# ChristianFeldmann/libHM

Hardware: AMD Instinct MI355X
Metric: decoded Mpixels/s (luma), 2160p Main10 reconstruction + loop filters (higher is better)
Workload: dtype int16 samples / int32 accumulate; 1 GPU; 3840x2160 Main10 lowdelay_P pictures, pre-parsed CTU metadata: prep+MC+dequant/IT/recon+deblock+SAO, batch of 16 independent pictures per step, inputs resident in HBM; sub_benchmark=full, streams=2, parallelism=frame-parallel, 1 process per GPU, no data-path collective

## Files before the change

libhm_amd/csrc/itx_core.h:

```cpp
#pragma once
#include "hmgpu_dev.h"

namespace hmgpu {

__host__ __device__ constexpr int cos64(int a) {
  constexpr int t[33] = {64, 90, 90, 90, 89, 88, 87, 85, 83, 82, 80, 78, 75, 73, 70, 67, 64,
                         61, 57, 54, 50, 46, 43, 38, 36, 31, 25, 22, 18, 13, 9,  4,  0};
  return t[a];
}
__host__ __device__ constexpr int tmat(int n_size, int k, int n) {
  const int a = ((2 * n + 1) * k * (32 / n_size)) & 127;
  return a <= 32 ? cos64(a) : (a <= 64 ? -cos64(64 - a) : (a <= 96 ? -cos64(a - 64) : cos64(128 - a)));
}
__host__ __device__ constexpr int dst4(int m, int k) {
  constexpr int t[4][4] = {{29, 55, 74, 84}, {74, 74, 0, -74}, {84, -29, -74, 55}, {55, -84, 74, -29}};
  return t[m][k];
}

__device__ inline void wave_lds_sync() {
  __builtin_amdgcn_fence(__ATOMIC_RELEASE, "wavefront");
  __builtin_amdgcn_wave_barrier();
  __builtin_amdgcn_fence(__ATOMIC_ACQUIRE, "wavefront");
}

typedef short short2v __attribute__((ext_vector_type(2)));
__host__ __device__ constexpr uint32_t pkc(int lo, int hi) { return ((uint32_t)lo & 0xffffu) | ((uint32_t)hi << 16); }

__host__ __device__ constexpr int slot_k(int n_size, int s) {
  int size = n_size / 2, g = 1, base = 0;
  while (size >= 1) {
    if (s < base + size) return (2 * (s - base) + 1) << (g - 1);
    base += size; size /= 2; g++;
  }
  return 0;
}
__host__ __device__ constexpr int slot_of_c(int n_size, int k) {
  for (int s = 0; s < n_size; s++) if (slot_k(n_size, s) == k) return s;
  return -1;
}
__device__ inline int slot_of(int n_size, int k) {
  if (k == 0) return n_size - 1;
  const int g = __builtin_ctz(k) + 1;
  return n_size - (n_size >> (g - 1)) + (k >> g);
}

__device__ inline int dot2c(uint32_t pair, uint32_t taps, int acc) {
  return __builtin_amdgcn_sdot2(__builtin_bit_cast(short2v, pair), __builtin_bit_cast(short2v, taps), acc, false);
}
__device__ inline int dot2_z(uint32_t pair, uint32_t taps) {
  int d;
  asm("v_dot2_i32_i16 %0, %1, %2, 0" : "=v"(d) : "v"(pair), "s"(taps));
  return d;
}
__device__ inline int dot2_v(uint32_t pair, uint32_t taps, int seed) {
  int d;
  asm("v_dot2_i32_i16 %0, %1, %2, %3" : "=v"(d) : "v"(pair), "s"(taps), "v"(seed));
  return d;
}
__device__ inline uint32_t pk_mad_sat(uint32_t a, uint32_t b) {
  uint32_t d;
  asm("v_pk_mad_i16 %0, %1, %2, 0 clamp" : "=v"(d) : "v"(a), "v"(b));
  return d;
}
__device__ inline uint32_t pk_add_sat(uint32_t a, uint32_t b) {
  uint32_t d;
  asm("v_pk_add_i16 %0, %1, %2 clamp" : "=v"(d) : "v"(a), "v"(b));
  return d;
}
__device__ inline uint32_t cvt_pk_sat(int lo, int hi) {
  uint32_t d;
  asm("v_cvt_pk_i16_i32 %0, %1, %2" : "=v"(d) : "v"(lo), "v"(hi));
  return d;
}
__device__ inline uint32_t pk_clip_u(uint32_t v, uint32_t hi) {
  const short2v z = {0, 0};
  const short2v r = __builtin_elementwise_min(__builtin_elementwise_max(__builtin_bit_cast(short2v, v), z), __builtin_bit_cast(short2v, hi));
  return __builtin_bit_cast(uint32_t, r);
}

template <int N, int OFF, int NP>
__device__ inline void idct_pk(const uint32_t (&p)[NP], int seed, int (&out)[N]) {
  if constexpr (N == 2) {
    out[0] = dot2_v(p[OFF], pkc(64, 64), seed);
    out[1] = dot2_v(p[OFF], pkc(-64, 64), seed);
  } else {
    int e[N / 2];
    idct_pk<N / 2, OFF + N / 4, NP>(p, seed, e);
#pragma unroll
    for (int m = 0; m < N / 2; m++) {
      int o = dot2_z(p[OFF], pkc(tmat(N, 1, m), tmat(N, 3, m)));
#pragma unroll
      for (int i = 1; i < N / 4; i++) o = dot2c(p[OFF + i], pkc(tmat(N, 4 * i + 1, m), tmat(N, 4 * i + 3, m)), o);
      out[m] = e[m] + o;
      out[N - 1 - m] = e[m] - o;
    }
  }
}

template <int LOG2N> struct PkCfg {
  static constexpr int N = 1 << LOG2N;
  static constexpr int S = N == 4 ? 4 : (N == 8 ? 24 : N + 8);
  static constexpr int TU_ELEMS = N * S + (N >= 16 ? 8 : 0);
  static constexpr int TPB = 256 / N;
};

template <int N, int S>
__device__ inline void scatter_row(int16_t* __restrict__ buf, int sn, const uint32_t (&v)[N / 2]) {
#pragma unroll
  for (int i = 0; i < N / 2; i++) {
    buf[(2 * i) * S + sn] = (int16_t)(v[i] & 0xffffu);
    buf[(2 * i + 1) * S + sn] = (int16_t)(v[i] >> 16);
  }
}
template <int N, int S>
__device__ inline void gather_row(const int16_t* __restrict__ buf, int n, uint32_t (&v)[N / 2]) {
  if constexpr (N == 4) {
    const u32x2 a = *reinterpret_cast<const u32x2*>(buf + n * S);
    v[0] = a.x; v[1] = a.y;
  } else {
#pragma unroll
    for (int i = 0; i < N / 8; i++) {
      const u32x4 a = *reinterpret_cast<const u32x4*>(buf + n * S + 8 * i);
      v[4 * i] = a.x; v[4 * i + 1] = a.y; v[4 * i + 2] = a.z; v[4 * i + 3] = a.w;
    }
  }
}
__device__ inline int half_of(uint32_t w, int hi) { return hi ? ((int)w >> 16) : (int)(int16_t)(w & 0xffffu); }

template <int N>
__device__ inline void idst4_pk(const uint32_t (&p)[N / 2], int seed, int (&out)[N]) {
  if constexpr (N == 4) {
#pragma unroll
    for (int k = 0; k < 4; k++) out[k] = dot2c(p[1], pkc(dst4(2, k), dst4(0, k)), dot2_v(p[0], pkc(dst4(1, k), dst4(3, k)), seed));
  }
}
template <int LOG2N>
__device__ inline void itx_tu_pk(const uint32_t (&lv)[(1 << LOG2N) / 2], int n, int per, int rem, bool skip, int bd,
                                 int16_t* __restrict__ buf, uint32_t (&res)[(1 << LOG2N) / 2], bool dst = false,
                                 const uint8_t* __restrict__ mrow = nullptr, bool bypass = false) {
  constexpr int N = 1 << LOG2N, S = PkCfg<LOG2N>::S;
  if (bypass) {
#pragma unroll
    for (int i = 0; i < N / 2; i++) res[i] = lv[i];
    return;
  }
  const int tshift = 15 - bd - LOG2N;
  const int rshift = 6 - (tshift + per);
  const int scale = rem == 0 ? 40 : rem == 1 ? 45 : rem == 2 ? 51 : rem == 3 ? 57 : rem == 4 ? 64 : 72;
  uint32_t d[N / 2];
  if (mrow != nullptr) {
    const int rs = rshift + 4;
    const int tb = min(16, 17 + rs), in_max = (1 << (tb - 1)) - 1, in_min = -in_max - 1;
    uint32_t mw[N / 4];
    if constexpr (N == 4) mw[0] = ldg(reinterpret_cast<const uint32_t*>(mrow));
    else {
#pragma unroll
      for (int i = 0; i < N / 16; i++) { const u32x4 a = ldg4(mrow + 16 * i); mw[4 * i] = a.x; mw[4 * i + 1] = a.y; mw[4 * i + 2] = a.z; mw[4 * i + 3] = a.w; }
      if constexpr (N == 8) { const u32x2 a = ldg2(mrow); mw[0] = a.x; mw[1] = a.y; }
    }
#pragma unroll
    for (int i = 0; i < N / 2; i++) {
      const int m0 = (mw[i / 2] >> (16 * (i & 1))) & 0xff, m1 = (mw[i / 2] >> (16 * (i & 1) + 8)) & 0xff;
      const int q0 = clip3(in_min, in_max, half_of(lv[i], 0)), q1 = clip3(in_min, in_max, half_of(lv[i], 1));
      int c0 = __mul24(q0, scale * m0), c1 = __mul24(q1, scale * m1);
      if (rs > 0) { c0 = (c0 + (1 << (rs - 1))) >> rs; c1 = (c1 + (1 << (rs - 1))) >> rs; }
      else { c0 = (int)((unsigned)c0 << (-rs)); c1 = (int)((unsigned)c1 << (-rs)); }
      d[i] = cvt_pk_sat(c0, c1);
    }
  } else if (rshift <= 0) {
    const uint32_t sp = (uint32_t)(scale << (-rshift)) * 0x10001u;
#pragma unroll
    for (int i = 0; i < N / 2; i++) d[i] = pk_mad_sat(lv[i], sp);
  } else {
    const int add = 1 << (rshift - 1);
#pragma unroll
    for (int i = 0; i < N / 2; i++)
      d[i] = cvt_pk_sat((__mul24(half_of(lv[i], 0), scale) + add) >> rshift, (__mul24(half_of(lv[i], 1), scale) + add) >> rshift);
  }
  const int sn = slot_of(N, n);
  scatter_row<N, S>(buf, sn, d);
  wave_lds_sync();
  uint32_t p[N / 2];
  gather_row<N, S>(buf, n, p);
  wave_lds_sync();
  uint32_t t1[N / 2];
  if (skip) {
    int o[N];
#pragma unroll
    for (int sidx = 0; sidx < N; sidx++) {
      const int c = half_of(p[sidx / 2], sidx & 1);
      o[slot_k(N, sidx)] = tshift > 0 ? (c + (1 << (tshift - 1))) >> tshift : (tshift == 0 ? c : c << (-tshift));
    }
#pragma unroll
    for (int i = 0; i < N / 2; i++) t1[i] = cvt_pk_sat(o[2 * i], o[2 * i + 1]);
  } else {
    int o[N];
    if (LOG2N == 2 && dst) idst4_pk<N>(p, 64, o);
    else idct_pk<N, 0, N / 2>(p, 64, o);
#pragma unroll
    for (int i = 0; i < N / 2; i++) t1[i] = cvt_pk_sat(o[2 * i] >> 7, o[2 * i + 1] >> 7);
  }
  scatter_row<N, S>(buf, sn, t1);
  wave_lds_sync();
  uint32_t q[N / 2];
  gather_row<N, S>(buf, n, q);
  wave_lds_sync();
  if (skip) {
#pragma unroll
    for (int i = 0; i < N / 2; i++) {
      constexpr int dummy = 0; (void)dummy;
      const int s0 = slot_of_c(N, 2 * i), s1 = slot_of_c(N, 2 * i + 1);
      res[i] = __builtin_amdgcn_perm(q[s1 / 2], q[s0 / 2], ((s1 & 1) ? 0x07060000u : 0x05040000u) | ((s0 & 1) ? 0x0302u : 0x0100u));
    }
  } else {
    const int shift2 = 20 - bd;
    int r[N];
    if (LOG2N == 2 && dst) idst4_pk<N>(q, 1 << (shift2 - 1), r);
    else idct_pk<N, 0, N / 2>(q, 1 << (shift2 - 1), r);
#pragma unroll
    for (int i = 0; i < N / 2; i++) res[i] = cvt_pk_sat(r[2 * i] >> shift2, r[2 * i + 1] >> shift2);
  }
}

template <int LOG2N>
__device__ inline void resid_rotate_rdpcm(uint32_t (&res)[(1 << LOG2N) / 2], int n, bool rotate, int rdpcm) {
  constexpr int N = 1 << LOG2N;
  typedef unsigned short u16x2 __attribute__((ext_vector_type(2)));
  if constexpr (N == 4) {
    if (rotate) {
      const uint32_t a = (uint32_t)__shfl_xor((int)res[1], 3), b = (uint32_t)__shfl_xor((int)res[0], 3);
      res[0] = (a >> 16) | (a << 16); res[1] = (b >> 16) | (b << 16);
    }
  }
  if (rdpcm == 1) {
    uint32_t carry = 0;
#pragma unroll
    for (int i = 0; i < N / 2; i++) {
      const uint32_t lo = (res[i] + carry) & 0xffffu, hi = ((res[i] >> 16) + lo) & 0xffffu;
      res[i] = lo | (hi << 16); carry = hi;
    }
  } else if (rdpcm == 2) {
#pragma unroll
    for (int d = 1; d < N; d <<= 1) {
#pragma unroll
      for (int i = 0; i < N / 2; i++) {
        const uint32_t up = (uint32_t)__shfl_up((int)res[i], d, N);
        const u16x2 s = __builtin_bit_cast(u16x2, res[i]) + __builtin_bit_cast(u16x2, up);
        if (n >= d) res[i] = __builtin_bit_cast(uint32_t, s);
      }
    }
  }
}

}
```

libhm_amd/csrc/k_itx.hip:

```cpp
#include "hmgpu_dev.h"
#include "itx_core.h"
#include <algorithm>

namespace hmgpu {

template <int LOG2N> struct ItxLds {
  static constexpr int BYTES = PkCfg<LOG2N>::TPB * PkCfg<LOG2N>::TU_ELEMS * 2;
};
constexpr int kItxLdsBytes = std::max(std::max(ItxLds<2>::BYTES, ItxLds<3>::BYTES), std::max(ItxLds<4>::BYTES, ItxLds<5>::BYTES));

struct ItxPic {
  const TuRec* list; uint32_t count_cap; const uint32_t* count;
  const int16_t* coef[3]; int16_t* resid[3]; int32_t rtw[3], bd[3]; const uint8_t* sl_m;
  int32_t csx, csy;
};
template <typename T> __device__ inline T by_comp(const T (&v)[3], int comp) { return comp == 0 ? v[0] : comp == 1 ? v[1] : v[2]; }

template <int LOG2N>
__device__ inline void itx_class(const ItxPic& P, int bx, int nbx, char* __restrict__ lds_raw) {
  constexpr int N = 1 << LOG2N;
  const TuRec* __restrict__ list = P.list;
  const uint32_t cap = P.count_cap;
  const int j = threadIdx.x / N, n = threadIdx.x % N;
  int16_t* buf = reinterpret_cast<int16_t*>(lds_raw) + j * PkCfg<LOG2N>::TU_ELEMS;
  constexpr int TPW = 64 / N;
  const int jw = (threadIdx.x & 63) / N;
  const uint32_t stride = (uint32_t)nbx * 4 * TPW;
  uint32_t t = ((uint32_t)bx * 4 + (threadIdx.x >> 6)) * TPW + jw;
  struct Rec { uint32_t w0, w1, w2; };
  auto load_rec = [&](uint32_t ti, Rec& r) {
    r.w0 = r.w1 = r.w2 = 0;
    if (ti < cap) { const uint32_t* rp = reinterpret_cast<const uint32_t*>(list + ti); r.w0 = ldg(rp); r.w1 = ldg(rp + 1); r.w2 = ldg(rp + 2); }
  };
  Rec rc, rn;
  load_rec(t, rc);
  load_rec(t + stride, rn);
  const uint32_t count = min(ldg(P.count), cap);
  auto load_levels = [&](uint32_t ti, const Rec& r, uint32_t (&lv)[N / 2]) {
#pragma unroll
    for (int i = 0; i < N / 2; i++) lv[i] = 0;
    if (ti < count) {
      const int16_t* lev = by_comp(P.coef, r.w1 & 3) + r.w2 + n * N;
      if constexpr (N == 4) { const u32x2 a = ldg2(lev); lv[0] = a.x; lv[1] = a.y; }
      else {
#pragma unroll
        for (int i = 0; i < N / 8; i++) { const u32x4 a = ldg4(lev + i * 8); lv[4 * i] = a.x; lv[4 * i + 1] = a.y; lv[4 * i + 2] = a.z; lv[4 * i + 3] = a.w; }
      }
    }
  };
  uint32_t lv_c[N / 2];
  load_levels(t, rc, lv_c);
  for (uint32_t tw = t - jw; tw < count; tw += stride, t += stride) {
    constexpr bool AHEAD = N < 32;
    uint32_t lv_n[AHEAD ? N / 2 : 1];
    Rec rnn;
    if constexpr (AHEAD) load_levels(t + stride, rn, lv_n);
    load_rec(t + 2 * stride, rnn);
    {
      const Rec r = rc;
      const int comp = r.w1 & 3, flags = (r.w1 & 0xff) >> 2;
      const int per = (int)(int8_t)((r.w1 >> 8) & 0xff), rem = (int)(int8_t)((r.w1 >> 16) & 0xff);
      const int bd = by_comp(P.bd, comp);
      uint32_t res[N / 2];
      const uint8_t* mrow = (P.sl_m != nullptr && (!(flags & 2) || N == 4)) ? P.sl_m + (((LOG2N - 2) * 6 + ((flags & 32) ? 0 : 3) + comp) << 10) + n * N : nullptr;
      itx_tu_pk<LOG2N>(lv_c, n, per, rem, (flags & 2) != 0, bd, buf, res, (flags & 1) != 0, mrow, (flags & 4) != 0);
      if ((flags & 0x18) | (r.w1 >> 24)) resid_rotate_rdpcm<LOG2N>(res, n, ((r.w1 >> 24) & 1) != 0, (flags >> 3) & 3);
      if (t < count) {
        const int x = ((int)(r.w0 & 0xffff) * 4) >> (comp ? P.csx : 0), y = ((((int)(r.w0 >> 16) * 4) >> (comp ? P.csy : 0))) + n;
        int16_t* row = by_comp(P.resid, comp) + ((size_t)((y >> 3) * by_comp(P.rtw, comp) + (x >> 3)) * 8 + resid_slot(y)) * 8;
        if constexpr (N == 4) stg2(row + (x & 4), u32x2{res[0], res[1]});
        else {
#pragma unroll
          for (int i = 0; i < N / 8; i++) stg4(row + i * 64, u32x4{res[4 * i], res[4 * i + 1], res[4 * i + 2], res[4 * i + 3]});
        }
      }
    }
    rc = rn; rn = rnn;
    if constexpr (AHEAD) {
#pragma unroll
      for (int i = 0; i < N / 2; i++) lv_c[i] = lv_n[i];
    } else {
      load_levels(t + stride, rc, lv_c);
    }
  }
}

__global__ void __launch_bounds__(256) k_itx(const ItxArgs a) {
  __shared__ __attribute__((aligned(16))) char lds[kItxLdsBytes];
  const int cls = blockIdx.y, shard = blockIdx.x & (kTuShards - 1), z = blockIdx.z;
  const int bx = blockIdx.x / kTuShards, nbx = a.blocks[cls];
  if (bx >= nbx) return;
  ItxPic P;
  P.list = a.tu[z][cls] + (size_t)shard * a.tu_cap[cls];
  P.count_cap = a.tu_cap[cls];
  P.count = a.tu_count[z] + cls * kTuShards + shard;
#pragma unroll
  for (int k = 0; k < 3; k++) { P.coef[k] = a.coef[z][k]; P.resid[k] = a.resid[z][k]; P.rtw[k] = a.rtw[k]; P.bd[k] = a.bd[k]; }
  P.sl_m = a.sl_m[z];
  P.csx = a.csx; P.csy = a.csy;
  switch (cls) {
    case 0: itx_class<2>(P, bx, nbx, lds); break;
    case 1: itx_class<3>(P, bx, nbx, lds); break;
    case 2: itx_class<4>(P, bx, nbx, lds); break;
    default: itx_class<5>(P, bx, nbx, lds); break;
  }
}

#ifndef ITX_B0
#define ITX_B0 1
#define ITX_B1 1
#define ITX_B2 1
#define ITX_B3 1
#endif
void launch_itx(ItxArgs& a, uint32_t blocks_per_shard, hipStream_t s) {
#ifdef ITX_BPS
  blocks_per_shard = ITX_BPS;
#endif
  const uint32_t div[4] = {ITX_B0, ITX_B1, ITX_B2, ITX_B3};
  for (int k = 0; k < 4; k++) a.blocks[k] = (a.class_mask >> k) & 1 ? (int32_t)std::max(1u, blocks_per_shard / div[k]) : 0;
  dim3 grid(blocks_per_shard * kTuShards, 4, (unsigned)a.n);
  hipLaunchKernelGGL(k_itx, grid, dim3(256), 0, s, a);
}

template <int LOG2N>
__global__ void __launch_bounds__(256) k_itx_flat(int bit_depth, int n_tus, const int16_t* __restrict__ levels,
                                                  const int8_t* __restrict__ per, const int8_t* __restrict__ rem,
                                                  const uint8_t* __restrict__ flags, int16_t* __restrict__ resid) {
  constexpr int N = 1 << LOG2N, TPB = PkCfg<LOG2N>::TPB;
  __shared__ __attribute__((aligned(16))) int16_t lds[TPB * PkCfg<LOG2N>::TU_ELEMS];
  const int j = threadIdx.x / N, n = threadIdx.x % N;
  for (int base = blockIdx.x * TPB; base < n_tus; base += gridDim.x * TPB) {
    const int t = base + j;
    const bool active = t < n_tus;
    uint32_t lv[N / 2], res[N / 2];
#pragma unroll
    for (int i = 0; i < N / 2; i++) lv[i] = active ? ldg(reinterpret_cast<const uint32_t*>(levels + (size_t)t * N * N + n * N) + i) : 0u;
    const int fl = active ? flags[t] : 0;
    itx_tu_pk<LOG2N>(lv, n, active ? per[t] : 0, active ? rem[t] : 0, (fl & 2) != 0, bit_depth, lds + j * PkCfg<LOG2N>::TU_ELEMS, res,
                     (fl & 1) != 0);
    if (!active) continue;
    uint32_t* row = reinterpret_cast<uint32_t*>(resid + (size_t)t * N * N + n * N);
#pragma unroll
    for (int i = 0; i < N / 2; i++) row[i] = res[i];
  }
}

void launch_itx_flat(int log2size, int bit_depth, int n, const int16_t* levels, const int8_t* per, const int8_t* rem,
                     const uint8_t* flags, int16_t* resid, hipStream_t s) {
  const int tpb = 256 >> log2size;
  dim3 grid((unsigned)std::min(4096, (n + tpb - 1) / tpb));
  switch (log2size) {
    case 2: hipLaunchKernelGGL(k_itx_flat<2>, grid, dim3(256), 0, s, bit_depth, n, levels, per, rem, flags, resid); break;
    case 3: hipLaunchKernelGGL(k_itx_flat<3>, grid, dim3(256), 0, s, bit_depth, n, levels, per, rem, flags, resid); break;
    case 4: hipLaunchKernelGGL(k_itx_flat<4>, grid, dim3(256), 0, s, bit_depth, n, levels, per, rem, flags, resid); break;
    case 5: hipLaunchKernelGGL(k_itx_flat<5>, grid, dim3(256), 0, s, bit_depth, n, levels, per, rem, flags, resid); break;
    default: break;
  }
}

}
```

Baseline: 182,000 Mpixels/s.

## Add 8x8 low-frequency corner fast path for 16x16 and 32x32 inverse transforms

For 16x16 and 32x32 TUs whose nonzero coefficients lie only in the top-left 8x8 corner across the whole wavefront, a reduced inverse transform runs. It does a truncated first pass using precomputed packed tap tables and a butterfly that prunes dead terms. Dequant is factored into a helper that handles only the live rows, and special modes (skip, bypass, rdpcm, rotate) fall back to the full path. Separately, the launch adds an amdgpu_waves_per_eu occupancy hint, which adds register pressure constraints and a wave-uniform branch whose benefit depends on how sparse the coefficients are.

```diff
diff --git a/libhm_amd/csrc/itx_core.h b/libhm_amd/csrc/itx_core.h
--- a/libhm_amd/csrc/itx_core.h
+++ b/libhm_amd/csrc/itx_core.h
@@ -127,6 +127,43 @@
 }
 __device__ inline int half_of(uint32_t w, int hi) { return hi ? ((int)w >> 16) : (int)(int16_t)(w & 0xffffu); }
 
+template <int LOG2N, int NR>
+__device__ inline void dequant_pk(const uint32_t (&lv)[(1 << LOG2N) / 2], int per, int rem, int bd, const uint8_t* __restrict__ mrow,
+                                  uint32_t (&d)[NR]) {
+  const int tshift = 15 - bd - LOG2N;
+  const int rshift = 6 - (tshift + per);
+  const int scale = rem == 0 ? 40 : rem == 1 ? 45 : rem == 2 ? 51 : rem == 3 ? 57 : rem == 4 ? 64 : 72;
+  if (mrow != nullptr) {
+    const int rs = rshift + 4;
+    const int tb = min(16, 17 + rs), in_max = (1 << (tb - 1)) - 1, in_min = -in_max - 1;
+    uint32_t mw[(NR + 1) / 2];
+    if constexpr (NR == 2) mw[0] = ldg(reinterpret_cast<const uint32_t*>(mrow));
+    else {
+#pragma unroll
+      for (int i = 0; i < NR / 8; i++) { const u32x4 a = ldg4(mrow + 16 * i); mw[4 * i] = a.x; mw[4 * i + 1] = a.y; mw[4 * i + 2] = a.z; mw[4 * i + 3] = a.w; }
+      if constexpr (NR == 4) { const u32x2 a = ldg2(mrow); mw[0] = a.x; mw[1] = a.y; }
+    }
+#pragma unroll
+    for (int i = 0; i < NR; i++) {
+      const int m0 = (mw[i / 2] >> (16 * (i & 1))) & 0xff, m1 = (mw[i / 2] >> (16 * (i & 1) + 8)) & 0xff;
+      const int q0 = clip3(in_min, in_max, half_of(lv[i], 0)), q1 = clip3(in_min, in_max, half_of(lv[i], 1));
+      int c0 = __mul24(q0, scale * m0), c1 = __mul24(q1, scale * m1);
+      if (rs > 0) { c0 = (c0 + (1 << (rs - 1))) >> rs; c1 = (c1 + (1 << (rs - 1))) >> rs; }
+      else { c0 = (int)((unsigned)c0 << (-rs)); c1 = (int)((unsigned)c1 << (-rs)); }
+      d[i] = cvt_pk_sat(c0, c1);
+    }
+  } else if (rshift <= 0) {
+    const uint32_t sp = (uint32_t)(scale << (-rshift)) * 0x10001u;
+#pragma unroll
+    for (int i = 0; i < NR; i++) d[i] = pk_mad_sat(lv[i], sp);
+  } else {
+    const int add = 1 << (rshift - 1);
+#pragma unroll
+    for (int i = 0; i < NR; i++)
+      d[i] = cvt_pk_sat((__mul24(half_of(lv[i], 0), scale) + add) >> rshift, (__mul24(half_of(lv[i], 1), scale) + add) >> rshift);
+  }
+}
+
 template <int N>
 __device__ inline void idst4_pk(const uint32_t (&p)[N / 2], int seed, int (&out)[N]) {
   if constexpr (N == 4) {
@@ -145,38 +182,8 @@
     return;
   }
   const int tshift = 15 - bd - LOG2N;
-  const int rshift = 6 - (tshift + per);
-  const int scale = rem == 0 ? 40 : rem == 1 ? 45 : rem == 2 ? 51 : rem == 3 ? 57 : rem == 4 ? 64 : 72;
   uint32_t d[N / 2];
-  if (mrow != nullptr) {
-    const int rs = rshift + 4;
-    const int tb = min(16, 17 + rs), in_max = (1 << (tb - 1)) - 1, in_min = -in_max - 1;
-    uint32_t mw[N / 4];
-    if constexpr (N == 4) mw[0] = ldg(reinterpret_cast<const uint32_t*>(mrow));
-    else {
-#pragma unroll
-      for (int i = 0; i < N / 16; i++) { const u32x4 a = ldg4(mrow + 16 * i); mw[4 * i] = a.x; mw[4 * i + 1] = a.y; mw[4 * i + 2] = a.z; mw[4 * i + 3] = a.w; }
-      if constexpr (N == 8) { const u32x2 a = ldg2(mrow); mw[0] = a.x; mw[1] = a.y; }
-    }
-#pragma unroll
-    for (int i = 0; i < N / 2; i++) {
-      const int m0 = (mw[i / 2] >> (16 * (i & 1))) & 0xff, m1 = (mw[i / 2] >> (16 * (i & 1) + 8)) & 0xff;
-      const int q0 = clip3(in_min, in_max, half_of(lv[i], 0)), q1 = clip3(in_min, in_max, half_of(lv[i], 1));
-      int c0 = __mul24(q0, scale * m0), c1 = __mul24(q1, scale * m1);
-      if (rs > 0) { c0 = (c0 + (1 << (rs - 1))) >> rs; c1 = (c1 + (1 << (rs - 1))) >> rs; }
-      else { c0 = (int)((unsigned)c0 << (-rs)); c1 = (int)((unsigned)c1 << (-rs)); }
-      d[i] = cvt_pk_sat(c0, c1);
-    }
-  } else if (rshift <= 0) {
-    const uint32_t sp = (uint32_t)(scale << (-rshift)) * 0x10001u;
-#pragma unroll
-    for (int i = 0; i < N / 2; i++) d[i] = pk_mad_sat(lv[i], sp);
-  } else {
-    const int add = 1 << (rshift - 1);
-#pragma unroll
-    for (int i = 0; i < N / 2; i++)
-      d[i] = cvt_pk_sat((__mul24(half_of(lv[i], 0), scale) + add) >> rshift, (__mul24(half_of(lv[i], 1), scale) + add) >> rshift);
-  }
+  dequant_pk<LOG2N, N / 2>(lv, per, rem, bd, mrow, d);
   const int sn = slot_of(N, n);
   scatter_row<N, S>(buf, sn, d);
   wave_lds_sync();
@@ -220,6 +227,105 @@
 #pragma unroll
     for (int i = 0; i < N / 2; i++) res[i] = cvt_pk_sat(r[2 * i] >> shift2, r[2 * i + 1] >> shift2);
   }
+}
+
+constexpr int kItxExtent = 8;
+
+template <int N> struct ItxCornerTaps {
+  alignas(16) uint32_t v[N][4];
+  constexpr ItxCornerTaps() : v{} {
+    for (int m = 0; m < N; m++)
+      for (int i = 0; i < 4; i++) v[m][i] = pkc(tmat(N, slot_k(8, 2 * i), m), tmat(N, slot_k(8, 2 * i + 1), m));
+  }
+};
+template <int N> struct ItxCornerTapsDev { static __device__ const ItxCornerTaps<N> tab; };
+template <int N> __device__ const ItxCornerTaps<N> ItxCornerTapsDev<N>::tab = ItxCornerTaps<N>();
+
+template <int N, int OFF, int NP, int G, int K>
+__device__ inline void idct_pk_lim(const uint32_t (&p)[NP], int seed, int (&out)[N]) {
+  if constexpr (N == 2) {
+    out[0] = dot2_v(p[OFF], pkc(64, 64), seed);
+    if constexpr (G < K) out[1] = dot2_v(p[OFF], pkc(-64, 64), seed);
+    else out[1] = out[0];
+  } else {
+    int e[N / 2];
+    idct_pk_lim<N / 2, OFF + N / 4, NP, 2 * G, K>(p, seed, e);
+    constexpr int live = G >= K ? 0 : ((K - 1) / G - 1) / 4 + 1 < N / 4 ? ((K - 1) / G - 1) / 4 + 1 : N / 4;
+#pragma unroll
+    for (int m = 0; m < N / 2; m++) {
+      if constexpr (live == 0) { out[m] = e[m]; out[N - 1 - m] = e[m]; }
+      else {
+        int o = dot2_z(p[OFF], pkc(tmat(N, 1, m), tmat(N, 3, m)));
+#pragma unroll
+        for (int i = 1; i < live; i++) o = dot2c(p[OFF + i], pkc(tmat(N, 4 * i + 1, m), tmat(N, 4 * i + 3, m)), o);
+        out[m] = e[m] + o;
+        out[N - 1 - m] = e[m] - o;
+      }
+    }
+  }
+}
+
+template <int LOG2N>
+__device__ inline void itx_tu_pk_corner(const uint32_t (&lv)[(1 << LOG2N) / 2], int n, int per, int rem, int bd,
+                                        int16_t* __restrict__ buf, uint32_t (&res)[(1 << LOG2N) / 2],
+                                        const uint8_t* __restrict__ mrow) {
+  constexpr int N = 1 << LOG2N, S = PkCfg<LOG2N>::S, K = kItxExtent;
+  static_assert(N >= 16 && K == 8, "corner form: 16x16 and 32x32 TUs, 8 x 8 corner");
+  asm volatile("" : "+v"(n));
+  const u32x4 tp = ldg4(&ItxCornerTapsDev<N>::tab.v[n][0]);
+  uint32_t d[K / 2];
+  dequant_pk<LOG2N, K / 2>(lv, per, rem, bd, mrow, d);
+  if (n < K) {
+    const int sn = slot_of(K, n);
+#pragma unroll
+    for (int i = 0; i < K / 2; i++) {
+      buf[(2 * i) * S + sn] = (int16_t)(d[i] & 0xffffu);
+      buf[(2 * i + 1) * S + sn] = (int16_t)(d[i] >> 16);
+    }
+  }
+  wave_lds_sync();
+  int o[K];
+#pragma unroll
+  for (int x = 0; x < K; x++) {
+    const u32x4 c = *reinterpret_cast<const u32x4*>(buf + x * S);
+    o[x] = dot2c(c.w, tp.w, dot2c(c.z, tp.z, dot2c(c.y, tp.y, dot2c(c.x, tp.x, 64)))) >> 7;
+  }
+  wave_lds_sync();
+  uint32_t q[N / 2];
+#pragma unroll
+  for (int i = 0; i < N / 2; i++) q[i] = 0;
+  q[0] = cvt_pk_sat(o[1], o[3]);
+  q[1] = cvt_pk_sat(o[5], o[7]);
+  q[N / 4] = cvt_pk_sat(o[2], o[6]);
+  q[N / 4 + N / 8] = cvt_pk_sat(o[4], 0);
+  q[N / 2 - 1] = cvt_pk_sat(0, o[0]);
+  const int shift2 = 20 - bd;
+  int r[N];
+  idct_pk_lim<N, 0, N / 2, 1, K>(q, 1 << (shift2 - 1), r);
+#pragma unroll
+  for (int i = 0; i < N / 2; i++) res[i] = cvt_pk_sat(r[2 * i] >> shift2, r[2 * i + 1] >> shift2);
+}
+
+template <int LOG2N>
+__device__ inline void itx_tu_pk_ext(const uint32_t (&lv)[(1 << LOG2N) / 2], int n, int per, int rem, bool skip, int bd,
+                                     int16_t* __restrict__ buf, uint32_t (&res)[(1 << LOG2N) / 2], bool dst,
+                                     const uint8_t* __restrict__ mrow, bool bypass, bool special) {
+#ifndef ITX_FULL_ONLY
+  if constexpr (LOG2N >= 4) {
+    constexpr int N = 1 << LOG2N, K = kItxExtent;
+    uint32_t hi = 0, lo = 0;
+#pragma unroll
+    for (int i = K / 2; i < N / 2; i++) hi |= lv[i];
+#pragma unroll
+    for (int i = 0; i < K / 2; i++) lo |= lv[i];
+    if (n >= K) hi |= lo;
+    if (!__any((hi != 0) | special)) {
+      itx_tu_pk_corner<LOG2N>(lv, n, per, rem, bd, buf, res, mrow);
+      return;
+    }
+  }
+#endif
+  itx_tu_pk<LOG2N>(lv, n, per, rem, skip, bd, buf, res, dst, mrow, bypass);
 }
 
 template <int LOG2N>
diff --git a/libhm_amd/csrc/k_itx.hip b/libhm_amd/csrc/k_itx.hip
--- a/libhm_amd/csrc/k_itx.hip
+++ b/libhm_amd/csrc/k_itx.hip
@@ -63,7 +63,8 @@
       const int bd = by_comp(P.bd, comp);
       uint32_t res[N / 2];
       const uint8_t* mrow = (P.sl_m != nullptr && (!(flags & 2) || N == 4)) ? P.sl_m + (((LOG2N - 2) * 6 + ((flags & 32) ? 0 : 3) + comp) << 10) + n * N : nullptr;
-      itx_tu_pk<LOG2N>(lv_c, n, per, rem, (flags & 2) != 0, bd, buf, res, (flags & 1) != 0, mrow, (flags & 4) != 0);
+      const bool special = t < count && (((flags & 0x1e) | (r.w1 >> 24)) != 0);
+      itx_tu_pk_ext<LOG2N>(lv_c, n, per, rem, (flags & 2) != 0, bd, buf, res, (flags & 1) != 0, mrow, (flags & 4) != 0, special);
       if ((flags & 0x18) | (r.w1 >> 24)) resid_rotate_rdpcm<LOG2N>(res, n, ((r.w1 >> 24) & 1) != 0, (flags >> 3) & 3);
       if (t < count) {
         const int x = ((int)(r.w0 & 0xffff) * 4) >> (comp ? P.csx : 0), y = ((((int)(r.w0 >> 16) * 4) >> (comp ? P.csy : 0))) + n;
@@ -85,7 +86,7 @@
   }
 }
 
-__global__ void __launch_bounds__(256) k_itx(const ItxArgs a) {
+__global__ void __launch_bounds__(256) __attribute__((amdgpu_waves_per_eu(6))) k_itx(const ItxArgs a) {
   __shared__ __attribute__((aligned(16))) char lds[kItxLdsBytes];
   const int cls = blockIdx.y, shard = blockIdx.x & (kTuShards - 1), z = blockIdx.z;
   const int bx = blockIdx.x / kTuShards, nbx = a.blocks[cls];
@@ -136,8 +137,8 @@
 #pragma unroll
     for (int i = 0; i < N / 2; i++) lv[i] = active ? ldg(reinterpret_cast<const uint32_t*>(levels + (size_t)t * N * N + n * N) + i) : 0u;
     const int fl = active ? flags[t] : 0;
-    itx_tu_pk<LOG2N>(lv, n, active ? per[t] : 0, active ? rem[t] : 0, (fl & 2) != 0, bit_depth, lds + j * PkCfg<LOG2N>::TU_ELEMS, res,
-                     (fl & 1) != 0);
+    itx_tu_pk_ext<LOG2N>(lv, n, active ? per[t] : 0, active ? rem[t] : 0, (fl & 2) != 0, bit_depth, lds + j * PkCfg<LOG2N>::TU_ELEMS, res,
+                         (fl & 1) != 0, nullptr, false, (fl & 2) != 0);
     if (!active) continue;
     uint32_t* row = reinterpret_cast<uint32_t*>(resid + (size_t)t * N * N + n * N);
 #pragma unroll
```

Result: no change. 181,600 Mpixels/s (-0.2%).
